# hwwang55/GraphGAN

Measured on NVIDIA B200. Metric: sampled negative edges/sec (D-sampling pass), higher is better.
Workload: dtype f32

## Files before the change

graphgan_b200/_cabi.py:

```python
import ctypes as C
import os

from . import _build

_LIB = None
ABI_VERSION = 3


class GGError(RuntimeError):
    pass


class WalkDesc(C.Structure):
    _fields_ = [
        ("n_node", C.c_int64), ("ld", C.c_int32),
        ("emb", C.c_void_p), ("bias", C.c_void_p), ("indptr", C.c_void_p), ("adj", C.c_void_p),
        ("n_roots", C.c_int64), ("roots", C.c_void_p), ("tree_bits", C.c_void_p), ("tree_words", C.c_int64),
        ("walk_ptr", C.c_void_p),
        ("n_walks", C.c_int64), ("for_d", C.c_int32), ("rng_mode", C.c_int32), ("d1_bits", C.c_void_p),
        ("seed", C.c_uint64), ("pass_tag", C.c_uint32), ("max_path", C.c_int32),
        ("stream", C.c_void_p), ("n_stream", C.c_int64), ("update_ratio", C.c_double),
        ("max_cand", C.c_int32), ("phase_mask", C.c_int32),
        ("samples", C.c_void_p), ("status", C.c_void_p), ("first_edge", C.c_void_p), ("wsteps", C.c_void_p),
        ("wsuml", C.c_void_p), ("paths", C.c_void_p), ("path_len", C.c_void_p), ("counters", C.c_void_p),
        ("scratch", C.c_void_p), ("scratch_bytes", C.c_int64), ("work_counter", C.c_void_p),
        ("edge_score", C.c_void_p), ("root_q", C.c_void_p), ("rq_ptr", C.c_void_p),
        ("hub_threshold", C.c_int32), ("no_tma", C.c_int32), ("walk_slot", C.c_void_p),
        ("s1_nq", C.c_int64), ("s1_slot", C.c_void_p), ("s1_ptr", C.c_void_p), ("s1_cnt", C.c_void_p), ("s1_n", C.c_void_p),
        ("s1_q", C.c_void_p), ("s1_ids", C.c_void_p), ("first_idx", C.c_void_p), ("s1_order", C.c_void_p), ("walk_order", C.c_void_p),
        ("flat_buf", C.c_void_p), ("flat_bytes", C.c_int64), ("flat_steps", C.c_int32), ("flat_reserved", C.c_int32),
    ]


_P, _I32, _I64, _F = C.c_void_p, C.c_int32, C.c_int64, C.c_float
SIGNATURES = {
    "gg_last_error": (C.c_char_p, []),
    "gg_abi_version": (C.c_int, []),
    "gg_hub_scores": (C.c_int, [_I64, _P, _P, _I32, _P, _P, _P, _P, _I32, _P, _P]),
    "gg_root_cdf": (C.c_int, [C.POINTER(WalkDesc), _P, _P, _P]),
    "gg_walk_scratch_bytes": (C.c_int, [_I32, C.POINTER(_I64)]),
    "gg_walk_flat_bytes": (C.c_int, [_I64, _I32, _I32, C.POINTER(_I64)]),
    "gg_walk_sample": (C.c_int, [C.POINTER(WalkDesc), _P]),
    "gg_walk_finalize": (C.c_int, [_I64, _P, _I32, _P, _P, _P, _P, _P, _P, _P, _P, _P, _P]),
    "gg_emit_d_rows": (C.c_int, [_I64, _P, _P, _P, _P, _P, _P, _P, _P, _P, _P, _P, _P]),
    "gg_bfs_scratch_bytes": (C.c_int, [_I64, _I64, C.POINTER(_I64)]),
    "gg_tree_words": (C.c_int, [_I64, C.POINTER(_I64)]),
    "gg_bfs_build": (C.c_int, [_I64, _I64, _P, _P, _I64, _P, _P, _I64, _P, _I64, _P]),
    "gg_reverse_entries": (C.c_int, [_I64, _I64, _P, _P, _P, _P, _P]),
    "gg_bfs_build_ex": (C.c_int, [_I64, _I64, _P, _P, _P, _I64, _P, _P, _I64, _P, _I64, C.c_float, C.c_int32, _P]),
    "gg_tree_parent": (C.c_int, [_I64, _P, _P, _I64, _P, _P, _I64, _P, _P]),
    "gg_pair_reward": (C.c_int, [_I64, _P, _P, _P, _P, _I32, _P, _P]),
    "gg_all_score": (C.c_int, [_I64, _P, _P, _I32, _P, _P]),
    "gg_pair_grad": (C.c_int, [_I32, _I32, _I32, _P, _P, _P, _P, _P, _I32, _F, _P, _P, _P, _P, _P, _P]),
    "gg_grad_buf_floats": (_I64, [_I32, _I32]),
    "gg_grad_merge": (C.c_int, [_I32, _I32, _I32, _P, _P, _P, _P, _P, _P, _P]),
    "gg_comm_unique_id": (C.c_int, [_P]),
    "gg_comm_init": (C.c_int, [_P, _I32, _I32, C.POINTER(C.c_void_p)]),
    "gg_comm_destroy": (C.c_int, [_P]),
    "gg_comm_info": (C.c_int, [_P, C.POINTER(_I32), C.POINTER(_I32), C.POINTER(_I32), C.POINTER(C.c_uint64)]),
# ... 58 lines not shown
```

graphgan_b200/csrc/walk.cu:

```cuda
#include <string.h>

#include "walk_common.cuh"

namespace gg {
namespace {

struct Rng {
    int mode;
    uint32_t k0, k1, tag;
    const double *stream;
    long long n_stream;
    long long cursor;
    int exhausted;
    __device__ __forceinline__ double draw(uint32_t root, uint32_t walk, uint32_t step) {
        if (mode == GG_RNG_PHILOX) {
            uint32_t a, b;
            philox4x32_10(root, walk, step, tag, k0, k1, a, b);
            return u53(a, b);
        }
        if (cursor >= n_stream) { exhausted = 1; return 0.0; }
        return stream[cursor++];
    }
};

// ... 208 lines not shown
            const double u = rng.draw((uint32_t)root, k, (uint32_t)step);
            if (rng.exhausted) { status = GG_NOTRUN; break; }
            idx = (n == 1) ? 0 : choose_index(sc, n, m, u, lane, sc != s_sc ? reinterpret_cast<double *>(s_sc) : nullptr);
            nxt = ids[idx];
            __syncwarp();
            cyc[2] += (unsigned int)(clock64() - t_c);
        }
        cyc[step == 0 ? 3 : (step == 1 ? 4 : 5)] += (unsigned int)(clock64() - t_step);
        if (step == 0) fedge = (int)(a0 + idx);
        if (prow && lane == 0 && plen < d.max_path) prow[plen] = nxt;
        ++plen;
        ++steps; suml += n;
        if (inc_father && idx == 0) { sample = cur; status = GG_DONE; break; }
        prev = cur; cur = nxt; ++step;
    }
    cyc[6] += (unsigned int)(clock64() - t_walk);
    raw_steps += (unsigned)(steps - steps_in); raw_suml += (unsigned)(suml - suml_in);
    if (lane == 0) {
        d.samples[w] = sample;
        d.status[w] = status;
        d.first_edge[w] = fedge;
        d.wsteps[w] = steps;
        d.wsuml[w] = suml;
        if (d.path_len) d.path_len[w] = (status == GG_DONE) ? plen : 0;
    }
    if (status == GG_DONE && d.max_path > 0 && plen > d.max_path) overflow += 1;
    return status;
}

__global__ void root_step_kernel(const __grid_constant__ gg_walk_desc d) {
    const long long w = (long long)blockIdx.x * blockDim.x + threadIdx.x;
    if (w >= d.n_walks) return;
    const int slot = __ldg(d.walk_slot + w);
    const int root = d.roots[slot];
    const uint32_t k = (uint32_t)(w - __ldg(d.walk_ptr + slot));
    const uint32_t k0 = (uint32_t)d.seed, k1 = (uint32_t)(d.seed >> 32);
    uint32_t a, b;
    if (d.update_ratio < 1.0) {
        philox4x32_10((uint32_t)root, 0xffffffffu, 0u, d.pass_tag, k0, k1, a, b);
        if (!(u53(a, b) < d.update_ratio)) { d.first_idx[w] = -2; return; }
    }
    const long long a0 = d.indptr[root];
    const int n = (int)(d.indptr[root + 1] - a0);
    if (n == 0) { d.first_idx[w] = -1; return; }
    philox4x32_10((uint32_t)root, k, 0u, d.pass_tag, k0, k1, a, b);
    const long long o = __ldg(d.rq_ptr + slot);
    const int idx = cdf_search(d.root_q + o, n, u53(a, b));
    d.first_idx[w] = idx;
    atomicAdd(d.s1_cnt + o + idx, 1);
}

constexpr int S1_SINGLES = 8192, S1_CHUNK = 16;

template <int CPL>
__global__ void __launch_bounds__(WARPS_PER_CTA * 32, WALK_MIN_CTAS) step1_cdf_kernel(const __grid_constant__ gg_walk_desc d) {
    extern __shared__ __align__(16) unsigned char walk_smem[];
    const int lane = threadIdx.x & 31, wid = threadIdx.x >> 5;
    float *s_sc = reinterpret_cast<float *>(walk_smem + (size_t)wid * WALK_SMEM_PER_WARP);
    int *s_ids = reinterpret_cast<int *>(s_sc + SC_CAP);
    Stage stg;
    stg.buf = s_sc;
    stg.bar = reinterpret_cast<unsigned long long *>(s_ids + ID_CAP);
    stg.phase = 0u;
    stg.on = !d.no_tma && d.edge_score != nullptr;
    if (stg.on) {
        if (lane == 0) {
            mbar_init(stg.bar, 1);
            asm volatile("fence.mbarrier_init.release.cluster;" ::: "memory");
        }
        __syncwarp();
    }
    const long long gw = (long long)blockIdx.x * WARPS_PER_CTA + wid;
    const long long nwarps = (long long)gridDim.x * WARPS_PER_CTA;
    int *g_ids = reinterpret_cast<int *>(d.scratch) + (size_t)gw * 2 * (size_t)d.max_cand;
    float *g_sc = reinterpret_cast<float *>(g_ids + d.max_cand);
    unsigned long long rows_gathered = 0;
    unsigned int cyc[7] = {0, 0, 0, 0, 0, 0, 0};
    long long item = gw, sub = 0, sub_end = 0;
    const long long n_single = d.s1_nq < S1_SINGLES ? d.s1_nq : S1_SINGLES;
    const long long n_items = n_single + (d.s1_nq - n_single + S1_CHUNK - 1) / S1_CHUNK;
    for (;;) {
        long long pos;
        if (d.s1_order) {
            if (sub >= sub_end) {
                unsigned int it = 0;
                if (lane == 0) it = atomicAdd(d.work_counter, 1u);
                it = __shfl_sync(FULL, it, 0);
                if ((long long)it >= n_items) break;
                if ((long long)it < n_single) { sub = it; sub_end = sub + 1; }
                else { sub = n_single + ((long long)it - n_single) * S1_CHUNK; sub_end = sub + S1_CHUNK < d.s1_nq ? sub + S1_CHUNK : d.s1_nq; }
            }
            pos = __ldg(d.s1_order + sub);
            ++sub;
        } else {
            if (item >= d.s1_nq) break;
            pos = item;
            item += nwarps;
        }
        if (!s1_is_shared(d, pos)) continue;
        const int slot = __ldg(d.s1_slot + pos);
        const int root = d.roots[slot];
        const uint32_t *tb = d.tree_bits + (size_t)slot * (size_t)d.tree_words;
        const long long e = d.indptr[root] + (pos - __ldg(d.rq_ptr + slot));
        const int c = __ldg(d.adj + e);
        const bool inc_father = !d.for_d && !((d.d1_bits[e >> 5] >> (e & 31)) & 1u);
        int n; float m; int *ids; float *sc;
        build_list<CPL, UNR_S1>(d, tb, c, root, inc_father, s_ids, s_sc, g_ids, g_sc, lane, n, m, ids, sc, rows_gathered, cyc, stg);
        if (lane == 0) d.s1_n[pos] = n;
        if (n == 0) continue;
        const long long o = __ldg(d.s1_ptr + pos);
        for (int i = lane; i < n; i += 32) d.s1_ids[o + i] = ids[i];
        if (n > 1) cdf_store_raw<UNR_S1>(sc, n, m, d.s1_q + o, lane);
        __syncwarp();
    }
    if (lane == 0 && rows_gathered) atomicAdd(d.counters + GG_CNT_ROWS_GATHERED, rows_gathered);
}

struct FlatView {
    int4 *list[2];
    int4 *tail;
    int *hub;
    int *item_n;
    int *pool_ids;
    unsigned *ctr;
    int stride;
    int steps;
};
constexpr int FLAT_MAX_STEPS = 14;
constexpr int FLAT_CTR_WORDS = 1 + 4 * (FLAT_MAX_STEPS + 2);
#define GG_FCTR(fv, s, k) ((fv).ctr + 1 + 4 * (s) + (k))

template <int CPL>
__global__ void __launch_bounds__(WARPS_PER_CTA * 32, WALK_MIN_CTAS) walk_kernel(const __grid_constant__ gg_walk_desc d,
                                                                                 const FlatView fv, const int tail_mode) {
    extern __shared__ __align__(16) unsigned char walk_smem[];
    const int lane = threadIdx.x & 31, wid = threadIdx.x >> 5;
    float *s_sc = reinterpret_cast<float *>(walk_smem + (size_t)wid * WALK_SMEM_PER_WARP);
    int *s_ids = reinterpret_cast<int *>(s_sc + SC_CAP);
    Stage stg;
    stg.buf = s_sc;
    stg.bar = reinterpret_cast<unsigned long long *>(s_ids + ID_CAP);
    stg.phase = 0u;
    stg.on = !d.no_tma && d.edge_score != nullptr;
    if (stg.on) {
        if (lane == 0) {
            mbar_init(stg.bar, 1);
            asm volatile("fence.mbarrier_init.release.cluster;" ::: "memory");
        }
        __syncwarp();
    }
    const long long gw = (long long)blockIdx.x * WARPS_PER_CTA + wid;
    int *g_ids = reinterpret_cast<int *>(d.scratch) + (size_t)gw * 2 * (size_t)d.max_cand;
    float *g_sc = reinterpret_cast<float *>(g_ids + d.max_cand);
    Rng rng;
    rng.mode = GG_RNG_PHILOX; rng.k0 = (uint32_t)d.seed; rng.k1 = (uint32_t)(d.seed >> 32); rng.tag = d.pass_tag;
    rng.stream = nullptr; rng.n_stream = 0; rng.cursor = 0; rng.exhausted = 0;
    unsigned long long raw_steps = 0, raw_suml = 0, overflow = 0, rows_gathered = 0;
    unsigned int cyc[7] = {0, 0, 0, 0, 0, 0, 0};
    const bool ratio_all = d.update_ratio >= 1.0;

    const long long n_items = tail_mode ? (long long)fv.ctr[0] : d.n_walks;
    for (;;) {
        unsigned int wi = 0;
        if (lane == 0) wi = atomicAdd(d.work_counter, 1u);
        wi = __shfl_sync(FULL, wi, 0);
        if ((long long)wi >= n_items) break;
        if (tail_mode) {
            const int4 rec = fv.tail[wi];
// ... 434 lines not shown
        const long long slot = walk_root_slot(walk_ptr, n_roots, w);
        if (!root_ok[slot]) continue;
        const int r = roots[slot];
        const long long w0 = walk_ptr[slot], k = walk_ptr[slot + 1] - w0, t = w - w0, o = row_ptr[slot];
        center[o + t] = r; neighbor[o + t] = pos_flat[pos_indptr[r] + t]; label[o + t] = 1;
        center[o + k + t] = r; neighbor[o + k + t] = samples[w]; label[o + k + t] = 0;
    }
}

int grid_ctas() { return sm_count() * WALK_MIN_CTAS; }

}
}

extern "C" int gg_walk_scratch_bytes(int32_t max_cand, int64_t *bytes) {
    GG_REQUIRE(bytes && max_cand > 0, "bad arguments");
    const int64_t warps = (int64_t)gg::grid_ctas() * gg::WARPS_PER_CTA;
    *bytes = warps * 2 * (int64_t)max_cand * 4;
    return 0;
}

extern "C" int gg_walk_flat_bytes(int64_t n_walks, int32_t hub_threshold, int32_t flat_steps, int64_t *bytes) {
    GG_REQUIRE(bytes && n_walks >= 0 && hub_threshold > 0 && flat_steps >= 0 && flat_steps <= gg::FLAT_MAX_STEPS, "bad arguments");
    *bytes = (int64_t)gg::flat_layout(nullptr, n_walks, hub_threshold, flat_steps, nullptr);
    return 0;
}

extern "C" int gg_walk_sample(const gg_walk_desc *dp, void *stream) {
    GG_REQUIRE(dp, "null descriptor");
    const gg_walk_desc &d = *dp;
    GG_REQUIRE(d.ld > 0 && d.ld % 32 == 0, "ld must be a positive multiple of 32");
    if (d.n_walks == 0 || d.n_roots == 0) return 0;
    GG_REQUIRE(d.emb && d.bias && d.indptr && d.adj && d.roots && d.tree_bits && d.walk_ptr, "null graph/embedding pointer");
    GG_REQUIRE(d.tree_words > 0, "tree_words missing (gg_tree_words)");
    GG_REQUIRE(d.samples && d.status && d.first_edge && d.wsteps && d.wsuml && d.counters && d.work_counter,
               "null output pointer");
    GG_REQUIRE(d.for_d || d.d1_bits, "G mode needs d1_bits");
    GG_REQUIRE(d.n_walks < (1ll << 32), "too many walks in one call");
    GG_REQUIRE(d.max_cand > 0 && d.scratch, "scratch missing");
    GG_REQUIRE(!d.root_q || d.rq_ptr, "root_q needs rq_ptr");
    GG_REQUIRE(d.max_path >= 0 && (d.max_path == 0 || (d.paths && d.path_len)), "max_path > 0 needs paths and path_len");
    GG_REQUIRE(d.phase_mask >= 0 && d.phase_mask <= 3, "phase_mask must be 0..3");
    GG_REQUIRE(d.update_ratio >= 0.0, "update_ratio must be >= 0");
    GG_REQUIRE(d.rng_mode == GG_RNG_PHILOX || d.rng_mode == GG_RNG_STREAM, "unknown rng_mode");
    {
        const bool any_s1 = d.s1_q || d.s1_ids || d.s1_cnt || d.s1_n || d.s1_ptr || d.s1_slot || d.first_idx || d.s1_order;
        GG_REQUIRE(!any_s1 || (d.s1_q && d.s1_ids && d.s1_cnt && d.s1_n && d.s1_ptr && d.s1_slot && d.first_idx && d.s1_nq > 0),
                   "depth-1 reuse: s1_q, s1_ids, s1_cnt, s1_n, s1_ptr, s1_slot, first_idx and s1_nq go together");
        GG_REQUIRE(!any_s1 || d.rng_mode == GG_RNG_PHILOX, "depth-1 reuse needs GG_RNG_PHILOX");
        GG_REQUIRE(!d.walk_order || d.rng_mode == GG_RNG_PHILOX, "walk_order needs GG_RNG_PHILOX");
    }
    GG_REQUIRE(!d.edge_score || (d.hub_threshold > 0 && d.hub_threshold < gg::SMEM_CAP), "hub_threshold out of range");
    cudaStream_t st = (cudaStream_t)stream;
    GG_CHECK(cudaMemsetAsync(d.work_counter, 0, sizeof(unsigned int), st));
    if (d.n_walks == 0 || d.n_roots == 0) return 0;
    const int cpl = d.ld / 32;
    if (d.rng_mode == GG_RNG_STREAM) {
        GG_REQUIRE(d.stream, "stream mode needs the uniform stream");
        GG_REQUIRE(d.scratch_bytes >= 2ll * d.max_cand * 4, "scratch too small");
        switch (cpl) {
#define GG_STREAM(C)                                                                                                  \
    GG_CHECK(cudaFuncSetAttribute(gg::walk_stream_kernel<C>, cudaFuncAttributeMaxDynamicSharedMemorySize,            \
                                  gg::WALK_SMEM_PER_WARP));                                                          \
    gg::walk_stream_kernel<C><<<1, 32, gg::WALK_SMEM_PER_WARP, st>>>(d)
            case 1: GG_STREAM(1); break;
            case 2: GG_STREAM(2); break;
            case 4: GG_STREAM(4); break;
            case 8: GG_STREAM(8); break;
#undef GG_STREAM
            default: gg::set_error("gg_walk_sample: unsupported ld %d (supported: 32, 64, 128, 256)", d.ld); return 2;
        }
    } else {
        const int ctas = gg::grid_ctas();
        GG_REQUIRE(d.scratch_bytes >= (int64_t)ctas * gg::WARPS_PER_CTA * 2 * d.max_cand * 4, "scratch too small");
        const int pm = d.phase_mask ? d.phase_mask : 3;
        if (d.s1_q && (pm & 1)) {
            GG_REQUIRE(d.root_q && d.walk_slot && d.first_idx && d.s1_cnt && d.s1_n && d.s1_ptr && d.s1_ids && d.s1_slot,
                       "depth-1 reuse needs root_q, walk_slot and the s1_* buffers");
            GG_CHECK(cudaMemsetAsync(d.s1_cnt, 0, sizeof(int32_t) * (size_t)d.s1_nq, st));
            gg::root_step_kernel<<<(unsigned)((d.n_walks + 255) / 256), 256, 0, st>>>(d);
            GG_CHECK(cudaGetLastError());
#define GG_S1(C)                                                                                                      \
    GG_CHECK(cudaFuncSetAttribute(gg::step1_cdf_kernel<C>, cudaFuncAttributeMaxDynamicSharedMemorySize,              \
                                  gg::WARPS_PER_CTA * gg::WALK_SMEM_PER_WARP));                                      \
    gg::step1_cdf_kernel<C><<<ctas, gg::WARPS_PER_CTA * 32, gg::WARPS_PER_CTA * gg::WALK_SMEM_PER_WARP, st>>>(d)
            switch (cpl) {
                case 1: GG_S1(1); break;
                case 2: GG_S1(2); break;
                case 4: GG_S1(4); break;
                case 8: GG_S1(8); break;
                default: gg::set_error("gg_walk_sample: unsupported ld %d (supported: 32, 64, 128, 256)", d.ld); return 2;
            }
#undef GG_S1
            GG_CHECK(cudaGetLastError());
            GG_CHECK(cudaMemsetAsync(d.work_counter, 0, sizeof(unsigned int), st));
        }
        if (!(pm & 2)) return 0;
        gg::FlatView fv;
        memset(&fv, 0, sizeof(fv));
        int tail_mode = 0;
        if (d.flat_steps > 0) {
            GG_REQUIRE(d.s1_q && d.edge_score && d.root_q && d.walk_slot && d.first_idx, "flat_steps needs the depth-1 reuse (s1_*, edge_score, root_q, walk_slot)");
            GG_REQUIRE(d.flat_steps <= gg::FLAT_MAX_STEPS, "flat_steps too large");
            GG_REQUIRE(d.flat_buf && d.flat_bytes >= (int64_t)gg::flat_layout(nullptr, d.n_walks, d.hub_threshold, d.flat_steps, nullptr),
                       "flat_buf too small (gg_walk_flat_bytes)");
            gg::flat_layout(d.flat_buf, d.n_walks, d.hub_threshold, d.flat_steps, &fv);
            GG_CHECK(cudaMemsetAsync(fv.ctr, 0, sizeof(unsigned) * gg::FLAT_CTR_WORDS, st));
// ... 83 lines not shown
```

graphgan_b200/csrc/walk_common.cuh:

```cuda
#pragma once
#include "gg_common.cuh"

namespace gg {

#ifndef GG_SC_CAP
#define GG_SC_CAP 1024
#endif
#ifndef GG_UNR
#define GG_UNR 2
#endif
#ifndef GG_UNR_S1
#define GG_UNR_S1 8
#endif
#ifndef GG_WALK_MIN_CTAS
#define GG_WALK_MIN_CTAS 4
#endif
constexpr int WARPS_PER_CTA = 8;
constexpr int WALK_MIN_CTAS = GG_WALK_MIN_CTAS;
constexpr int ID_CAP = 320;
constexpr int SC_CAP = GG_SC_CAP;
constexpr int SMEM_CAP = ID_CAP;
constexpr int WALK_SMEM_PER_WARP = SC_CAP * 4 + ID_CAP * 4 + 16;
constexpr int STAGE_ENTRIES = 512;
static_assert(2 * STAGE_ENTRIES * 4 <= SC_CAP * 4, "the staging area is the warp's (idle) score buffer");
// ... 40 lines not shown
#pragma unroll
        for (int c = 0; c < CPL; ++c) sb = fma4(c4[c], xb[c], sb);
        sa = group8_sum(sa);
        sb = group8_sum(sb);
        if (g == 0) {
            if (va) sc[ia] = __fadd_rn(sa, ba);
            if (vb) sc[ib] = __fadd_rn(sb, bb);
        }
    }
    __syncwarp();
}

template <int CPL>
__device__ __forceinline__ void score_edges(const float *__restrict__ emb, const float *__restrict__ bias, int ld,
                                            const float4 (&c4)[CPL], const int *__restrict__ adj, long long e0,
                                            int n, float *out, int fallback, int lane) {
    const int grp = lane >> 3, g = lane & 7;
    int ca_n = (grp < n) ? __ldg(adj + e0 + grp) : fallback, cb_n = (4 + grp < n) ? __ldg(adj + e0 + 4 + grp) : fallback;
    for (int i0 = 0; i0 < n; i0 += 8) {
        const int ia = i0 + grp, ib = i0 + 4 + grp;
        const bool va = ia < n, vb = ib < n;
        const int ca = ca_n, cb = cb_n;
        ca_n = (ia + 8 < n) ? __ldg(adj + e0 + ia + 8) : fallback;
        cb_n = (ib + 8 < n) ? __ldg(adj + e0 + ib + 8) : fallback;
        const float *ra = emb + (size_t)ca * (size_t)ld + 4 * g;
        const float *rb = emb + (size_t)cb * (size_t)ld + 4 * g;
        float4 xa[CPL], xb[CPL];
#pragma unroll
        for (int c = 0; c < CPL; ++c) xa[c] = ldg4(ra + 32 * c);
#pragma unroll
        for (int c = 0; c < CPL; ++c) xb[c] = ldg4(rb + 32 * c);
        const float ba = __ldg(bias + ca), bb = __ldg(bias + cb);
        float sa = 0.0f, sb = 0.0f;
#pragma unroll
        for (int c = 0; c < CPL; ++c) sa = fma4(c4[c], xa[c], sa);
#pragma unroll
        for (int c = 0; c < CPL; ++c) sb = fma4(c4[c], xb[c], sb);
        sa = group8_sum(sa);
        sb = group8_sum(sb);
        if (g == 0) {
            if (va) out[ia] = __fadd_rn(sa, ba);
            if (vb) out[ib] = __fadd_rn(sb, bb);
        }
    }
    __syncwarp();
}

__device__ __forceinline__ float list_max(const float *sc, int n, int lane) {
    float m = -INFINITY;
    for (int i = lane; i < n; i += 32) m = fmaxf(m, sc[i]);
    return warp_max(m);
}

template <int U = UNR>
__device__ __forceinline__ float softmax_exp_sum(float *sc, int n, float m, int lane) {
    float S = 0.0f;
    for (int t0 = 0; t0 < n; t0 += 32 * U) {
        float x[U];
#pragma unroll
        for (int u = 0; u < U; ++u) { const int i = t0 + 32 * u + lane; x[u] = (i < n) ? sc[i] : 0.0f; }
#pragma unroll
        for (int u = 0; u < U; ++u) {
            if (t0 + 32 * u >= n) break;
            const int i = t0 + 32 * u + lane;
            float e = 0.0f;
            if (i < n) { e = exp_c(__fsub_rn(x[u], m)); sc[i] = e; }
            S = __fadd_rn(S, warp_sum_butterfly(e));
        }
    }
    __syncwarp();
    return S;
}

template <int U = UNR>
__device__ __forceinline__ double cdf_total(const float *sc, int n, float S, int lane, double (&car)[2]) {
    double total = 0.0;
    car[0] = car[1] = 0.0;
    for (int t0 = 0; t0 < n; t0 += 32 * U) {
        float e[U];
#pragma unroll
        for (int u = 0; u < U; ++u) { const int i = t0 + 32 * u + lane; e[u] = (i < n) ? sc[i] : 0.0f; }
#pragma unroll
        for (int u = 0; u < U; ++u) {
            if (t0 + 32 * u >= n) break;
            double x = (double)__fdiv_rn(e[u], S);
            x = warp_scan_ks(x, lane);
            total = __dadd_rn(total, __shfl_sync(FULL, x, 31));
            const int t = (t0 >> 5) + u;
            if (t < 64 && lane == (t & 31)) car[t >> 5] = total;
        }
    }
    return total;
}

__device__ __forceinline__ int cdf_pick_from(const float *sc, int n, float S, double total, double u, int lane,
                                             int t_begin, double carry) {
    for (int t0 = 32 * t_begin; t0 < n; t0 += 32) {
        const int i = t0 + lane;
        double x = (double)__fdiv_rn((i < n) ? sc[i] : 0.0f, S);
        x = warp_scan_ks(x, lane);
        const double q = __ddiv_rn(__dadd_rn(carry, x), total);
        const unsigned hit = __ballot_sync(FULL, (i < n) && (q > u));
        if (hit) return t0 + __ffs(hit) - 1;
        carry = __dadd_rn(carry, __shfl_sync(FULL, x, 31));
    }
    return n - 1;
}

__device__ __forceinline__ int cdf_pick(const float *sc, int n, float S, double total, double u, int lane,
                                        const double (&car)[2]) {
    const int ntiles = (n + 31) >> 5;
    int t_hit = -1;
#pragma unroll
    for (int h = 0; h < 2; ++h) {
        const int t = 32 * h + lane;
        const bool p = (t < ntiles) && (__ddiv_rn(car[h], total) > u);
        const unsigned mk = __ballot_sync(FULL, p);
        if (t_hit < 0 && mk) t_hit = 32 * h + __ffs(mk) - 1;
    }
    if (t_hit < 0) {
        if (ntiles <= 64) return n - 1;
        const double c63 = __shfl_sync(FULL, car[1], 31);
        return cdf_pick_from(sc, n, S, total, u, lane, 64, c63);
    }
    double before = 0.0;
    if (t_hit > 0) {
        const int tp = t_hit - 1;
        const double lo = __shfl_sync(FULL, car[0], tp & 31), hi = __shfl_sync(FULL, car[1], tp & 31);
        before = (tp >> 5) ? hi : lo;
    }
    return cdf_pick_from(sc, n, S, total, u, lane, t_hit, before);
}

__device__ __forceinline__ double cdf_total_tiles(const float *sc, int n, float S, int lane, double *tiles) {
    constexpr int U = 8;
    double total = 0.0;
    for (int t0 = 0; t0 < n; t0 += 32 * U) {
        float e[U];
#pragma unroll
        for (int u = 0; u < U; ++u) { const int i = t0 + 32 * u + lane; e[u] = (i < n) ? sc[i] : 0.0f; }
#pragma unroll
        for (int u = 0; u < U; ++u) {
            if (t0 + 32 * u >= n) break;
            double x = (double)__fdiv_rn(e[u], S);
            x = warp_scan_ks(x, lane);
            total = __dadd_rn(total, __shfl_sync(FULL, x, 31));
            if (lane == 0) tiles[(t0 >> 5) + u] = total;
        }
    }
    __syncwarp();
    return total;
}
__device__ __forceinline__ int cdf_pick_tiles(const float *sc, int n, float S, double total, double u, int lane,
                                              const double *tiles) {
    const int ntiles = (n + 31) >> 5;
    for (int tb = 0; tb < ntiles; tb += 32) {
        const int t = tb + lane;
        const bool p = (t < ntiles) && (__ddiv_rn(tiles[t], total) > u);
        const unsigned mk = __ballot_sync(FULL, p);
        if (mk) {
            const int t_hit = tb + __ffs(mk) - 1;
            return cdf_pick_from(sc, n, S, total, u, lane, t_hit, t_hit > 0 ? tiles[t_hit - 1] : 0.0);
        }
    }
    return n - 1;
}

static __device__ __noinline__ int choose_index_long(float *sc, int n, float m, double u, int lane, double *tiles) {
    float S;
    double car[2], total;
    if (tiles && ((n + 31) >> 5) <= SC_CAP / 2) {
        S = softmax_exp_sum<8>(sc, n, m, lane);
        total = cdf_total_tiles(sc, n, S, lane, tiles);
        return cdf_pick_tiles(sc, n, S, total, u, lane, tiles);
    }
    S = softmax_exp_sum<8>(sc, n, m, lane);
    total = cdf_total<8>(sc, n, S, lane, car);
    return cdf_pick(sc, n, S, total, u, lane, car);
}

__device__ __forceinline__ int choose_index(float *sc, int n, float m, double u, int lane, double *tiles = nullptr) {
    if (n <= 32) {
        const float e = (lane < n) ? exp_c(__fsub_rn(sc[lane], m)) : 0.0f;
        const float S = warp_sum_butterfly(e);
        const double x = warp_scan_ks((double)__fdiv_rn(e, S), lane);
        const double total = __shfl_sync(FULL, x, 31);
        const unsigned hit = __ballot_sync(FULL, (lane < n) && (__ddiv_rn(x, total) > u));
        return hit ? __ffs(hit) - 1 : n - 1;
    }
    if (n > SC_CAP) return choose_index_long(sc, n, m, u, lane, tiles);
    double car[2];
    const float S = softmax_exp_sum(sc, n, m, lane);
    const double total = cdf_total(sc, n, S, lane, car);
    return cdf_pick(sc, n, S, total, u, lane, car);
}

__device__ __forceinline__ void cdf_store(float *sc, int n, double *q_out, int lane) {
    const float m = list_max(sc, n, lane);
    const float S = softmax_exp_sum<UNR_S1>(sc, n, m, lane);
    double car[2];
// ... 56 lines not shown
```

graphgan_b200/sampler.py:

```python
import ctypes as C
import os

import numpy as np

from . import _cabi
from ._cabi import ptr

RNG_PHILOX, RNG_STREAM = 0, 1
NOTRUN, DONE, VOID, SKIPPED = 0, 1, 2, 3
CNT = dict(steps=0, sum_l=1, accepted=2, ok_roots=3, path_overflow=4, raw_steps=5, raw_sum_l=6, stream_used=7,
           rows_gathered=8, cyc_enum=9, cyc_score=10, cyc_choose=11, cyc_step0=12, cyc_step1=13, cyc_step2p=14, cyc_walk=15)


def round_up(x, m):
    return (x + m - 1) // m * m


def pad_embedding(emb, device=None):
    import torch
    e = emb.float() if isinstance(emb, torch.Tensor) else torch.as_tensor(np.asarray(emb, np.float64).astype(np.float32))
    n, d = e.shape
    if d > 256:
        raise ValueError("n_emb = %d is not supported (the kernels are instantiated for row strides 32, 64, 128, 256)" % d)
    ld = 32
    while ld < d:
        ld *= 2
    out = torch.zeros((n, ld), dtype=torch.float32, device=device if device is not None else e.device)
    out[:, :d] = e.to(out.device)
    return out


class TreeBatch:

    def __init__(self, roots, tree_bits, graph=None):
        self.roots = roots
        self.tree_bits = tree_bits
        self.graph = graph

    def slice(self, lo, hi):
        return TreeBatch(self.roots[lo:hi].contiguous(), self.tree_bits[lo:hi].contiguous(), self.graph)

    def select(self, idx):
        return TreeBatch(self.roots[idx].contiguous(), self.tree_bits[idx].contiguous(), self.graph)

    def parent_arrays(self, rows=None):
        import torch
        g, lib = self.graph, _cabi.lib()
        bits = self.tree_bits if rows is None else self.tree_bits[rows].contiguous()
        roots = self.roots if rows is None else self.roots[rows].contiguous()
        R = int(bits.shape[0])
        out = torch.empty((R, g.n_node), dtype=torch.int32, device=bits.device)
        st = torch.cuda.current_stream(bits.device).cuda_stream
        for lo in range(0, R, 32768):
            hi = min(R, lo + 32768)
            _cabi.check(lib.gg_tree_parent(g.n_node, ptr(g.indptr), ptr(g.adj), hi - lo, ptr(roots[lo:hi]), ptr(bits[lo:hi]),
                                           int(bits.shape[1]), ptr(out[lo:hi]), st), "gg_tree_parent")
        return out


class WalkOutput:

    def __init__(self, **kw):
        self.__dict__.update(kw)

    def counters_host(self):
        c = self.counters.cpu().numpy().astype(np.uint64)
        return {k: int(c[i]) for k, i in CNT.items()}


class WalkPlan:

    def __init__(self, sampler, trees, sample_num, for_d, max_path):
        import torch
        dev, g = sampler.device, sampler.g
        R = int(trees.roots.shape[0])
        self.trees, self.for_d, self.max_path, self.n_roots = trees, bool(for_d), int(max_path), R
        if isinstance(sample_num, int):
            self.walk_ptr = torch.arange(R + 1, dtype=torch.int64, device=dev) * sample_num
            self.n_walks = R * sample_num
        else:
            self.walk_ptr = torch.zeros(R + 1, dtype=torch.int64, device=dev)
            self.walk_ptr[1:] = torch.cumsum(sample_num.to(torch.int64), 0)
            self.n_walks = int(self.walk_ptr[-1].item())
        nw = self.walk_ptr[1:] - self.walk_ptr[:-1]
        self.walk_slot = torch.repeat_interleave(torch.arange(R, dtype=torch.int32, device=dev), nw,
                                                 output_size=self.n_walks) if self.n_walks else None
        r = trees.roots.long()
        self.rq_ptr = torch.zeros(R + 1, dtype=torch.int64, device=dev)
        self.rq_ptr[1:] = torch.cumsum(g.indptr[r + 1] - g.indptr[r], 0)
        self.nq = int(self.rq_ptr[-1].item())
        nq = max(self.nq, 1)
        self.root_q = torch.empty(nq, dtype=torch.float64, device=dev)
        self.root_sc = torch.empty(nq, dtype=torch.float32, device=dev)
        self._s1 = None
        self._order = None
        W = max(self.n_walks, 1)
        i32 = lambda *s: torch.empty(s, dtype=torch.int32, device=dev)
        self.samples, self.status, self.first_edge, self.wsteps, self.wsuml = i32(W), i32(W), i32(W), i32(W), i32(W)
        self.paths = i32(W, max_path) if max_path > 0 else None
        self.path_len = i32(W) if max_path > 0 else None
        self.root_ok = torch.zeros(max(R, 1), dtype=torch.int32, device=dev)
        self.counters = torch.zeros(16, dtype=torch.int64, device=dev)
        self.row_ptr = torch.empty(R + 1, dtype=torch.int64, device=dev)
        self.n_rows = torch.zeros(1, dtype=torch.int64, device=dev)
        self.rows = [i32(max(2 * self.n_walks, 1)) for _ in range(3)] if for_d else None


    def start_order(self, sampler):
        if self._order is None and self.n_walks > 0 and self.nq > 0:
            torch, g, dev = sampler.torch, sampler.g, sampler.device
            R = self.n_roots
            deg_r = self.rq_ptr[1:] - self.rq_ptr[:-1]
            slot = torch.repeat_interleave(torch.arange(R, dtype=torch.int64, device=dev), deg_r, output_size=self.nq)
            ent = g.indptr[self.trees.roots.long()[slot]] + (torch.arange(self.nq, dtype=torch.int64, device=dev) - self.rq_ptr[slot])
            c = g.adj[ent].long()
            key = torch.zeros(R, dtype=torch.int64, device=dev).scatter_reduce_(0, slot, g.indptr[c + 1] - g.indptr[c], "amax")
            perm = torch.argsort(key, descending=True, stable=True)
            nw = (self.walk_ptr[1:] - self.walk_ptr[:-1])[perm]
            first = torch.cumsum(nw, 0) - nw
            base = torch.repeat_interleave(self.walk_ptr[:-1][perm] - first, nw, output_size=self.n_walks)
            self._order = (base + torch.arange(self.n_walks, dtype=torch.int64, device=dev)).to(torch.int32)
        return self._order

    def flat_buffer(self, sampler):
        key = (sampler.flat_steps, sampler.hub_threshold)
        if getattr(self, "_flat_key", None) != key:
            nbytes = C.c_int64(0)
            _cabi.check(sampler.lib.gg_walk_flat_bytes(self.n_walks, sampler.hub_threshold, sampler.flat_steps, C.byref(nbytes)),
                        "gg_walk_flat_bytes")
            self._flat = sampler.torch.empty(max(nbytes.value, 16), dtype=sampler.torch.uint8, device=sampler.device)
            self._flat_key = key
        return self._flat

    def depth1_buffers(self, sampler):
        if self._s1 is None:
            torch, g, dev = sampler.torch, sampler.g, sampler.device
            deg_r = self.rq_ptr[1:] - self.rq_ptr[:-1]
            slot = torch.repeat_interleave(torch.arange(self.n_roots, dtype=torch.int32, device=dev), deg_r, output_size=self.nq)
            r = self.trees.roots.long()[slot.long()]
            ent = g.indptr[r] + (torch.arange(self.nq, dtype=torch.int64, device=dev) - self.rq_ptr[slot.long()])
            c = g.adj[ent].long()
            ptr_ = torch.zeros(self.nq + 1, dtype=torch.int64, device=dev)
            ptr_[1:] = torch.cumsum(g.indptr[c + 1] - g.indptr[c] + 1, 0)
            total = max(int(ptr_[-1].item()), 1)
            i32 = lambda k: torch.empty(max(k, 1), dtype=torch.int32, device=dev)
            order = torch.argsort(g.indptr[c + 1] - g.indptr[c], descending=True, stable=True).to(torch.int32)
            self._s1 = dict(slot=slot, ptr=ptr_, cnt=i32(self.nq), n=i32(self.nq), ids=i32(total), order=order,
                            q=torch.empty(total, dtype=torch.float64, device=dev), first=i32(self.n_walks))
        return self._s1


class WalkSampler:
    def __init__(self, graph, hub_threshold=128, depth1=True, hub_first=True, tma=True):
        import torch
        self.torch = torch
        self.g = graph
        self.device = graph.device
        self.lib = _cabi.lib()
        self.max_cand = graph.max_deg + 1
        self.hub_threshold = int(hub_threshold)
        self.depth1 = bool(depth1)
        self.tma = bool(tma)
        self.hub_first = bool(hub_first)
        nbytes = C.c_int64(0)
        _cabi.check(self.lib.gg_walk_scratch_bytes(self.max_cand, C.byref(nbytes)), "gg_walk_scratch_bytes")
        self.scratch = torch.empty(max(nbytes.value, 16), dtype=torch.uint8, device=self.device)
        self.work_counter = torch.zeros(1, dtype=torch.int32, device=self.device)
        self._bfs_scratch = None
        self.bfs_bottom_up_ratio = float(os.environ.get("GG_BFS_BU_RATIO", "-1"))
        self.bfs_flags = 0
        self.flat_steps = int(os.environ.get("GG_FLAT_STEPS", "4"))

    def _stream(self):
        return self.torch.cuda.current_stream(self.device).cuda_stream

    def build_trees(self, roots):
        torch = self.torch
        roots_d = roots if isinstance(roots, torch.Tensor) else torch.as_tensor(np.asarray(roots, np.int32)).to(self.device)
        R, N = int(roots_d.shape[0]), self.g.n_node
        nnz = int(self.g.adj.shape[0])
        words = C.c_int64(0)
        _cabi.check(self.lib.gg_tree_words(nnz, C.byref(words)), "gg_tree_words")
        tree_bits = torch.empty((R, words.value), dtype=torch.int32, device=self.device)
        if self._bfs_scratch is None:
            nbytes = C.c_int64(0)
            _cabi.check(self.lib.gg_bfs_scratch_bytes(N, int(self.g.adj.shape[0]), C.byref(nbytes)), "gg_bfs_scratch_bytes")
            self._bfs_scratch = torch.empty(max(nbytes.value, 16), dtype=torch.uint8, device=self.device)
        rev = self.g.reverse_entries() if self.bfs_bottom_up_ratio != 0.0 else None
        _cabi.check(self.lib.gg_bfs_build_ex(N, nnz, ptr(self.g.indptr), ptr(self.g.adj), ptr(rev) if rev is not None else None,
                                             R, ptr(roots_d), ptr(tree_bits), words.value, ptr(self._bfs_scratch),
                                             self._bfs_scratch.numel(), float(self.bfs_bottom_up_ratio), int(self.bfs_flags),
                                             self._stream()),
                    "gg_bfs_build_ex")
        return TreeBatch(roots_d, tree_bits, self.g)

    def plan(self, trees, sample_num, for_d, max_path=0):
        return WalkPlan(self, trees, sample_num, for_d, max_path)

    def _desc(self, emb, bias, plan, *, seed, pass_tag, update_ratio, rng_mode, stream, reuse, phase_mask=0):
        torch = self.torch
        assert emb.dtype == torch.float32 and emb.is_contiguous() and bias.dtype == torch.float32
        t, d = plan.trees, _cabi.WalkDesc()
        d.n_node, d.ld = self.g.n_node, int(emb.shape[1])
        d.emb, d.bias, d.indptr, d.adj = ptr(emb), ptr(bias), ptr(self.g.indptr), ptr(self.g.adj)
        d.n_roots, d.roots, d.walk_ptr, d.n_walks = plan.n_roots, ptr(t.roots), ptr(plan.walk_ptr), plan.n_walks
        d.tree_bits, d.tree_words = ptr(t.tree_bits), int(t.tree_bits.shape[1])
        d.for_d, d.rng_mode, d.d1_bits = int(plan.for_d), rng_mode, ptr(self.g.d1_bits)
        d.seed, d.pass_tag, d.max_path = seed, pass_tag, plan.max_path
        d.stream, d.n_stream = (ptr(stream), int(stream.numel())) if stream is not None else (None, 0)
        d.update_ratio, d.max_cand, d.phase_mask = float(update_ratio), self.max_cand, int(phase_mask)
        d.no_tma = 0 if self.tma else 1
        d.samples, d.status, d.first_edge, d.wsteps, d.wsuml = (ptr(plan.samples), ptr(plan.status), ptr(plan.first_edge),
                                                                 ptr(plan.wsteps), ptr(plan.wsuml))
        d.paths, d.path_len, d.counters = ptr(plan.paths), ptr(plan.path_len), ptr(plan.counters)
        d.scratch, d.scratch_bytes, d.work_counter = ptr(self.scratch), self.scratch.numel(), ptr(self.work_counter)
        d.rq_ptr, d.walk_slot = ptr(plan.rq_ptr), ptr(plan.walk_slot)
        if self.hub_first and rng_mode == RNG_PHILOX:
            d.walk_order = ptr(plan.start_order(self))
        if reuse:
            self.g.hub_tiles(self.hub_threshold)
# ... 56 lines not shown
```

include/graphgan_b200.h:

```cpp
#ifndef GRAPHGAN_B200_H
#define GRAPHGAN_B200_H
#include <stdint.h>

#ifdef __cplusplus
extern "C" {
#endif

#define GG_ABI_VERSION 3

enum { GG_NOTRUN = 0, GG_DONE = 1, GG_VOID = 2, GG_SKIPPED = 3 };
enum {
    GG_RNG_PHILOX = 0,
    GG_RNG_STREAM = 1
};
enum {
    GG_CNT_STEPS = 0, GG_CNT_SUML = 1, GG_CNT_ACCEPTED = 2, GG_CNT_OK_ROOTS = 3,
    GG_CNT_PATH_OVERFLOW = 4, GG_CNT_RAW_STEPS = 5, GG_CNT_RAW_SUML = 6, GG_CNT_STREAM_USED = 7,
    GG_CNT_ROWS_GATHERED = 8,
    GG_CNT_CYC_ENUM = 9, GG_CNT_CYC_SCORE = 10, GG_CNT_CYC_CHOOSE = 11, GG_CNT_CYC_STEP0 = 12,
    GG_CNT_CYC_STEP1 = 13, GG_CNT_CYC_STEP2P = 14, GG_CNT_CYC_WALK = 15,
    GG_CNT_SLOTS = 16
};

const char *gg_last_error(void);
int gg_abi_version(void);

typedef struct gg_walk_desc {
    int64_t n_node;
    int32_t ld;
    const float *emb;
    const float *bias;
    const int64_t *indptr;
    const int32_t *adj;
    int64_t n_roots;
    const int32_t *roots;
    const uint32_t *tree_bits;
    int64_t tree_words;
    const int64_t *walk_ptr;
    int64_t n_walks;
    int32_t for_d;
    int32_t rng_mode;
    uint32_t *d1_bits;
    uint64_t seed;
    uint32_t pass_tag;
    int32_t max_path;
    const double *stream;
    int64_t n_stream;
    double update_ratio;
    int32_t max_cand;
    int32_t phase_mask;
    int32_t *samples;
    int32_t *status;
    int32_t *first_edge;
    int32_t *wsteps;
    int32_t *wsuml;
    int32_t *paths;
    int32_t *path_len;
    unsigned long long *counters;
    void *scratch;
    int64_t scratch_bytes;
    unsigned int *work_counter;
    const float *edge_score;
    const double *root_q;
    const int64_t *rq_ptr;
    int32_t hub_threshold;
    int32_t no_tma;
    const int32_t *walk_slot;
    int64_t s1_nq;
    const int32_t *s1_slot;
    const int64_t *s1_ptr;
    int32_t *s1_cnt;
    int32_t *s1_n;
    double *s1_q;
    int32_t *s1_ids;
// ... 117 lines not shown
```

Before: 120.2 million.

## Build step-1 CDFs for very large neighbor lists cooperatively across a whole CTA

Adds a CTA-cooperative phase in step1_cdf_kernel. Before the per-warp loop, whole blocks claim step-1 items whose neighbor list has at least 2048 entries (via a second work counter) and build their softmax CDF together: they count tree bits per warp, enumerate and score in parallel, then reduce and scan tiles in shared memory. The per-warp path then skips those lists. Separately, the per-warp softmax sum and CDF tile totals switch from one shuffle reduction per 32-element tile to a transposed multi-tile reduction, which needs fewer shuffles. The extra phase adds __syncthreads and a serial thread-0 loop over tiles, moves the mbarrier location in shared memory, and changes the float summation order.

Result: faster. 128.8 million, median of 6 (+7.2%).

```diff
diff --git a/graphgan_b200/_cabi.py b/graphgan_b200/_cabi.py
--- a/graphgan_b200/_cabi.py
+++ b/graphgan_b200/_cabi.py
@@ -4,7 +4,7 @@
 from . import _build
 
 _LIB = None
-ABI_VERSION = 3
+ABI_VERSION = 4
 
 
 class GGError(RuntimeError):
diff --git a/graphgan_b200/csrc/walk.cu b/graphgan_b200/csrc/walk.cu
--- a/graphgan_b200/csrc/walk.cu
+++ b/graphgan_b200/csrc/walk.cu
@@ -284,15 +284,191 @@
 
 constexpr int S1_SINGLES = 8192, S1_CHUNK = 16;
 
+#ifndef GG_CTA_LIST_MIN
+#define GG_CTA_LIST_MIN 2048
+#endif
+constexpr int CTA_LIST_MIN = GG_CTA_LIST_MIN;
+constexpr int CTA_SMEM = WARPS_PER_CTA * (SC_CAP + ID_CAP) * 4;
+constexpr int CTA_G = 8;
+static_assert(CTA_LIST_MIN >= ID_CAP, "CTA lists must be score-cached (hub_threshold < ID_CAP)");
+static_assert(CTA_SMEM + WARPS_PER_CTA * 8 <= WARPS_PER_CTA * WALK_SMEM_PER_WARP, "step1_cdf_kernel layout: buffers, then mbarriers");
+
+__device__ __forceinline__ bool cta_list(const gg_walk_desc &d, long long len) {
+    const long long groups = (len + 1 + 32 * CTA_G - 1) / (32 * CTA_G);
+    return d.edge_score && len >= CTA_LIST_MIN && groups * CTA_G * 8 <= CTA_SMEM;
+}
+
+struct CtaCtl {
+    long long a0, a1, o;
+    int pos, slot, cur, prev, inc_father;
+    int wcnt[WARPS_PER_CTA];
+    float wmax[WARPS_PER_CTA];
+    float S;
+};
+
+template <int CPL>
+__device__ __noinline__ void cta_build_cdf(const gg_walk_desc &d, CtaCtl &ctl, unsigned char *smem, float *g_sc, int lane,
+                                              int wid, unsigned long long &rows_gathered) {
+    const long long a0 = ctl.a0, a1 = ctl.a1;
+    const int f = ctl.inc_father;
+    const uint32_t *tb = d.tree_bits + (size_t)ctl.slot * (size_t)d.tree_words;
+    int *ids = d.s1_ids + ctl.o;
+    double *c_out = d.s1_q + ctl.o;
+    const long long wfirst = a0 >> 5, wlast = (a1 - 1) >> 5;
+    const long long per = (wlast - wfirst + WARPS_PER_CTA) / WARPS_PER_CTA;
+    const long long e_lo = max(a0, (wfirst + wid * per) << 5), e_hi = min(a1, (wfirst + (wid + 1) * per) << 5);
+    int cnt = 0;
+    if (e_lo < e_hi) {
+        const long long wl0 = e_lo >> 5, wl1 = (e_hi - 1) >> 5;
+        for (long long wb = wl0; wb <= wl1; wb += 32) {
+            const long long wi = wb + lane;
+            unsigned word = (wi <= wl1) ? __ldg(tb + wi) : 0u;
+            if (wi == wl0) word &= 0xffffffffu << (e_lo & 31);
+            if (wi == wl1 && (e_hi & 31)) word &= (1u << (e_hi & 31)) - 1u;
+            cnt += (int)__reduce_add_sync(FULL, (unsigned)__popc(word));
+        }
+    }
+    if (lane == 0) ctl.wcnt[wid] = cnt;
+    __syncthreads();
+    int off = f, n = f;
+#pragma unroll
+    for (int w = 0; w < WARPS_PER_CTA; ++w) {
+        const int c = ctl.wcnt[w];
+        if (w < wid) off += c;
+        n += c;
+    }
+    const int ntiles = (n + 31) >> 5;
+    double *tt = reinterpret_cast<double *>(smem);
+    float *sc = ((long long)ntiles * 8 + (long long)n * 4 <= CTA_SMEM) ? reinterpret_cast<float *>(smem + (size_t)ntiles * 8) : g_sc;
+    float m = -INFINITY;
+    if (e_lo < e_hi) {
+        Stage plain;
+        plain.buf = nullptr; plain.bar = nullptr; plain.phase = 0u; plain.on = false;
+        int nloc = 0;
+        enumerate_children<UNR_S1>(d, tb, e_lo, e_hi, true, ids + off, sc + off, lane, nloc, m, plain);
+    }
+    m = warp_max(m);
+    if (f && wid == 0) {
+        if (lane == 0) ids[0] = ctl.prev;
+        if (n > 1) {
+            float4 c4[CPL];
+            load_row<CPL>(d.emb, d.ld, ctl.cur, lane & 7, c4);
+            score_list<CPL>(d.emb, d.bias, d.ld, c4, &ctl.prev, sc, 1, ctl.cur, lane);
+            rows_gathered += 2;
+            m = fmaxf(m, sc[0]);
+        }
+    }
+    if (lane == 0) ctl.wmax[wid] = m;
+    __syncthreads();
+    if (n <= 1) {
+        if (threadIdx.x == 0) d.s1_n[ctl.pos] = n;
+        return;
+    }
+#pragma unroll
+    for (int w = 0; w < WARPS_PER_CTA; ++w) m = fmaxf(m, ctl.wmax[w]);
+    const int ngroups = (ntiles + CTA_G - 1) / CTA_G;
+    float *tsum = reinterpret_cast<float *>(smem);
+    for (int g = wid; g < ngroups; g += WARPS_PER_CTA) {
+        const int i0 = g * 32 * CTA_G;
+        float e[CTA_G];
+#pragma unroll
+        for (int u = 0; u < CTA_G; ++u) { const int i = i0 + 32 * u + lane; e[u] = (i < n) ? sc[i] : 0.0f; }
+#pragma unroll
+        for (int u = 0; u < CTA_G; ++u) {
+            const int i = i0 + 32 * u + lane;
+            if (i < n) { e[u] = exp_c(__fsub_rn(e[u], m)); sc[i] = e[u]; }
+        }
+        const float T = tile_sums<CTA_G>(e, lane);
+        const int t = g * CTA_G + lane / (32 / CTA_G);
+        if (lane % (32 / CTA_G) == 0 && t < ntiles) tsum[t] = T;
+    }
+    __syncthreads();
+    if (threadIdx.x == 0) {
+        float S = 0.0f;
+        for (int t = 0; t < ntiles; ++t) S = __fadd_rn(S, tsum[t]);
+        ctl.S = S;
+    }
+    __syncthreads();
+    const float S = ctl.S;
+    for (int g = wid; g < ngroups; g += WARPS_PER_CTA) {
+        const int i0 = g * 32 * CTA_G;
+        double x[CTA_G];
+#pragma unroll
+        for (int u = 0; u < CTA_G; ++u) { const int i = i0 + 32 * u + lane; x[u] = (double)__fdiv_rn((i < n) ? sc[i] : 0.0f, S); }
+        const double U = tile_totals<CTA_G>(x, lane);
+        const int t = g * CTA_G + tile_total_lane<CTA_G>(lane & (CTA_G - 1));
+        if (lane < CTA_G && t < ntiles) tt[t] = U;
+    }
+    __syncthreads();
+    if (threadIdx.x == 0) {
+        double C = 0.0;
+        for (int t = 0; t < ntiles; ++t) { C = __dadd_rn(C, tt[t]); tt[t] = C; }
+        c_out[n] = C;
+    }
+    __syncthreads();
+    for (int g = wid; g < ngroups; g += WARPS_PER_CTA) {
+        const int i0 = g * 32 * CTA_G;
+        double x[CTA_G];
+#pragma unroll
+        for (int u = 0; u < CTA_G; ++u) { const int i = i0 + 32 * u + lane; x[u] = (i < n) ? (double)__fdiv_rn(sc[i], S) : 0.0; }
+#pragma unroll
+        for (int u = 0; u < CTA_G; ++u) x[u] = warp_scan_ks(x[u], lane);
+#pragma unroll
+        for (int u = 0; u < CTA_G; ++u) {
+            const int t = g * CTA_G + u, i = i0 + 32 * u + lane;
+            if (i < n) c_out[i] = __dadd_rn(t > 0 ? tt[t - 1] : 0.0, x[u]);
+        }
+    }
+    if (threadIdx.x == 0) d.s1_n[ctl.pos] = n;
+}
+
+template <int CPL>
+__device__ __noinline__ unsigned long long cta_phase_run(const gg_walk_desc &d, unsigned char *walk_smem, int lane, int wid,
+                                                       unsigned long long &rows_gathered) {
+    __shared__ CtaCtl ctl;
+    unsigned long long cta_lists = 0;
+    float *cta_sc = reinterpret_cast<float *>(reinterpret_cast<int *>(d.scratch) +
+                                              (size_t)blockIdx.x * WARPS_PER_CTA * 2 * (size_t)d.max_cand + d.max_cand);
+    for (;;) {
+        if (threadIdx.x == 0) {
+            int pos = -1;
+            for (;;) {
+                const unsigned it = atomicAdd(d.work_counter + 1, 1u);
+                if ((long long)it >= d.s1_nq) break;
+                const int p = __ldg(d.s1_order + it);
+                const int slot = __ldg(d.s1_slot + p);
+                const int root = d.roots[slot];
+                const long long e = d.indptr[root] + (p - __ldg(d.rq_ptr + slot));
+                const int c = __ldg(d.adj + e);
+                const long long a0 = d.indptr[c], a1 = d.indptr[c + 1];
+                if (a1 - a0 < CTA_LIST_MIN) break;
+                if (!cta_list(d, a1 - a0) || !s1_is_shared(d, p)) continue;
+                ctl.a0 = a0; ctl.a1 = a1; ctl.o = __ldg(d.s1_ptr + p);
+                ctl.slot = slot; ctl.cur = c; ctl.prev = root;
+                ctl.inc_father = !d.for_d && !((d.d1_bits[e >> 5] >> (e & 31)) & 1u);
+                pos = p;
+                break;
+            }
+            ctl.pos = pos;
+        }
+        __syncthreads();
+        if (ctl.pos < 0) break;
+        cta_build_cdf<CPL>(d, ctl, walk_smem, cta_sc, lane, wid, rows_gathered);
+        cta_lists += 1;
+        __syncthreads();
+    }
+    return cta_lists;
+}
+
 template <int CPL>
 __global__ void __launch_bounds__(WARPS_PER_CTA * 32, WALK_MIN_CTAS) step1_cdf_kernel(const __grid_constant__ gg_walk_desc d) {
     extern __shared__ __align__(16) unsigned char walk_smem[];
     const int lane = threadIdx.x & 31, wid = threadIdx.x >> 5;
-    float *s_sc = reinterpret_cast<float *>(walk_smem + (size_t)wid * WALK_SMEM_PER_WARP);
+    float *s_sc = reinterpret_cast<float *>(walk_smem + (size_t)wid * (SC_CAP + ID_CAP) * 4);
     int *s_ids = reinterpret_cast<int *>(s_sc + SC_CAP);
     Stage stg;
     stg.buf = s_sc;
-    stg.bar = reinterpret_cast<unsigned long long *>(s_ids + ID_CAP);
+    stg.bar = reinterpret_cast<unsigned long long *>(walk_smem + CTA_SMEM) + wid;
     stg.phase = 0u;
     stg.on = !d.no_tma && d.edge_score != nullptr;
     if (stg.on) {
@@ -306,8 +482,10 @@
     const long long nwarps = (long long)gridDim.x * WARPS_PER_CTA;
     int *g_ids = reinterpret_cast<int *>(d.scratch) + (size_t)gw * 2 * (size_t)d.max_cand;
     float *g_sc = reinterpret_cast<float *>(g_ids + d.max_cand);
-    unsigned long long rows_gathered = 0;
+    unsigned long long rows_gathered = 0, cta_lists = 0;
     unsigned int cyc[7] = {0, 0, 0, 0, 0, 0, 0};
+    const bool cta_phase = d.s1_order && d.edge_score;
+    if (cta_phase) cta_lists = cta_phase_run<CPL>(d, walk_smem, lane, wid, rows_gathered);
     long long item = gw, sub = 0, sub_end = 0;
     const long long n_single = d.s1_nq < S1_SINGLES ? d.s1_nq : S1_SINGLES;
     const long long n_items = n_single + (d.s1_nq - n_single + S1_CHUNK - 1) / S1_CHUNK;
@@ -335,6 +513,7 @@
         const uint32_t *tb = d.tree_bits + (size_t)slot * (size_t)d.tree_words;
         const long long e = d.indptr[root] + (pos - __ldg(d.rq_ptr + slot));
         const int c = __ldg(d.adj + e);
+        if (cta_phase && cta_list(d, d.indptr[c + 1] - d.indptr[c])) continue;
         const bool inc_father = !d.for_d && !((d.d1_bits[e >> 5] >> (e & 31)) & 1u);
         int n; float m; int *ids; float *sc;
         build_list<CPL, UNR_S1>(d, tb, c, root, inc_father, s_ids, s_sc, g_ids, g_sc, lane, n, m, ids, sc, rows_gathered, cyc, stg);
@@ -346,6 +525,7 @@
         __syncwarp();
     }
     if (lane == 0 && rows_gathered) atomicAdd(d.counters + GG_CNT_ROWS_GATHERED, rows_gathered);
+    if (threadIdx.x == 0 && cta_lists) atomicAdd(d.counters + GG_CNT_CTA_LISTS, cta_lists);
 }
 
 struct FlatView {
@@ -886,7 +1066,7 @@
     }
     GG_REQUIRE(!d.edge_score || (d.hub_threshold > 0 && d.hub_threshold < gg::SMEM_CAP), "hub_threshold out of range");
     cudaStream_t st = (cudaStream_t)stream;
-    GG_CHECK(cudaMemsetAsync(d.work_counter, 0, sizeof(unsigned int), st));
+    GG_CHECK(cudaMemsetAsync(d.work_counter, 0, 2 * sizeof(unsigned int), st));
     if (d.n_walks == 0 || d.n_roots == 0) return 0;
     const int cpl = d.ld / 32;
     if (d.rng_mode == GG_RNG_STREAM) {
diff --git a/graphgan_b200/csrc/walk_common.cuh b/graphgan_b200/csrc/walk_common.cuh
--- a/graphgan_b200/csrc/walk_common.cuh
+++ b/graphgan_b200/csrc/walk_common.cuh
@@ -116,21 +116,68 @@
     return warp_max(m);
 }
 
+template <int G, typename T, typename Add>
+__device__ __forceinline__ T transposed_levels(T (&v)[G], int lane, int o0, bool down, Add add) {
+    static_assert(G >= 1 && G <= 32 && (G & (G - 1)) == 0, "G must be a power of two <= 32");
+    int o = o0;
+#pragma unroll
+    for (int k = G; k > 1; k >>= 1) {
+        const bool up = (lane & o) != 0;
+#pragma unroll
+        for (int j = 0; j < k / 2; ++j) {
+            const T send = up ? v[j] : v[j + k / 2];
+            const T keep = up ? v[j + k / 2] : v[j];
+            v[j] = add(keep, __shfl_xor_sync(FULL, send, o));
+        }
+        o = down ? (o >> 1) : (o << 1);
+    }
+    return v[0];
+}
+
+template <int G>
+__device__ __forceinline__ float tile_sums(float (&v)[G], int lane) {
+    const auto add = [](float a, float b) { return __fadd_rn(a, b); };
+    float s = transposed_levels<G>(v, lane, 16, true, add);
+#pragma unroll
+    for (int o = 16 / G; o >= 1; o >>= 1) s = __fadd_rn(s, __shfl_xor_sync(FULL, s, o));
+    return s;
+}
+template <int G>
+__device__ __forceinline__ constexpr int tile_sum_lane(int u) { return u * (32 / G); }
+
+template <int G>
+__device__ __forceinline__ double tile_totals(double (&v)[G], int lane) {
+    const auto add = [](double a, double b) { return __dadd_rn(a, b); };
+    double s = transposed_levels<G>(v, lane, 1, false, add);
+#pragma unroll
+    for (int o = G; o < 32; o <<= 1) s = __dadd_rn(s, __shfl_xor_sync(FULL, s, o));
+    return s;
+}
+template <int G>
+__device__ __forceinline__ constexpr int tile_total_lane(int u) {
+    int r = 0;
+    for (int b = 1, rb = G >> 1; b < G; b <<= 1, rb >>= 1) if (u & b) r |= rb;
+    return r;
+}
+
 template <int U = UNR>
 __device__ __forceinline__ float softmax_exp_sum(float *sc, int n, float m, int lane) {
     float S = 0.0f;
     for (int t0 = 0; t0 < n; t0 += 32 * U) {
-        float x[U];
-#pragma unroll
-        for (int u = 0; u < U; ++u) { const int i = t0 + 32 * u + lane; x[u] = (i < n) ? sc[i] : 0.0f; }
-#pragma unroll
-        for (int u = 0; u < U; ++u) {
-            if (t0 + 32 * u >= n) break;
+        float e[U];
+#pragma unroll
+        for (int u = 0; u < U; ++u) { const int i = t0 + 32 * u + lane; e[u] = (i < n) ? sc[i] : 0.0f; }
+#pragma unroll
+        for (int u = 0; u < U; ++u) {
             const int i = t0 + 32 * u + lane;
-            float e = 0.0f;
-            if (i < n) { e = exp_c(__fsub_rn(x[u], m)); sc[i] = e; }
-            S = __fadd_rn(S, warp_sum_butterfly(e));
-        }
+            if (i < n) { e[u] = exp_c(__fsub_rn(e[u], m)); sc[i] = e[u]; }
+        }
+        const float T = tile_sums<U>(e, lane);
+        float Tu[U];
+#pragma unroll
+        for (int u = 0; u < U; ++u) Tu[u] = __shfl_sync(FULL, T, tile_sum_lane<U>(u));
+#pragma unroll
+        for (int u = 0; u < U; ++u) S = __fadd_rn(S, Tu[u]);
     }
     __syncwarp();
     return S;
@@ -141,15 +188,16 @@
     double total = 0.0;
     car[0] = car[1] = 0.0;
     for (int t0 = 0; t0 < n; t0 += 32 * U) {
-        float e[U];
-#pragma unroll
-        for (int u = 0; u < U; ++u) { const int i = t0 + 32 * u + lane; e[u] = (i < n) ? sc[i] : 0.0f; }
-#pragma unroll
-        for (int u = 0; u < U; ++u) {
-            if (t0 + 32 * u >= n) break;
-            double x = (double)__fdiv_rn(e[u], S);
-            x = warp_scan_ks(x, lane);
-            total = __dadd_rn(total, __shfl_sync(FULL, x, 31));
+        double x[U];
+#pragma unroll
+        for (int u = 0; u < U; ++u) { const int i = t0 + 32 * u + lane; x[u] = (double)__fdiv_rn((i < n) ? sc[i] : 0.0f, S); }
+        const double Ut = tile_totals<U>(x, lane);
+        double Uu[U];
+#pragma unroll
+        for (int u = 0; u < U; ++u) Uu[u] = __shfl_sync(FULL, Ut, tile_total_lane<U>(u));
+#pragma unroll
+        for (int u = 0; u < U; ++u) {
+            total = __dadd_rn(total, Uu[u]);
             const int t = (t0 >> 5) + u;
             if (t < 64 && lane == (t & 31)) car[t >> 5] = total;
         }
@@ -200,16 +248,17 @@
     constexpr int U = 8;
     double total = 0.0;
     for (int t0 = 0; t0 < n; t0 += 32 * U) {
-        float e[U];
-#pragma unroll
-        for (int u = 0; u < U; ++u) { const int i = t0 + 32 * u + lane; e[u] = (i < n) ? sc[i] : 0.0f; }
-#pragma unroll
-        for (int u = 0; u < U; ++u) {
-            if (t0 + 32 * u >= n) break;
-            double x = (double)__fdiv_rn(e[u], S);
-            x = warp_scan_ks(x, lane);
-            total = __dadd_rn(total, __shfl_sync(FULL, x, 31));
-            if (lane == 0) tiles[(t0 >> 5) + u] = total;
+        double x[U];
+#pragma unroll
+        for (int u = 0; u < U; ++u) { const int i = t0 + 32 * u + lane; x[u] = (double)__fdiv_rn((i < n) ? sc[i] : 0.0f, S); }
+        const double Ut = tile_totals<U>(x, lane);
+        double Uu[U];
+#pragma unroll
+        for (int u = 0; u < U; ++u) Uu[u] = __shfl_sync(FULL, Ut, tile_total_lane<U>(u));
+#pragma unroll
+        for (int u = 0; u < U; ++u) {
+            total = __dadd_rn(total, Uu[u]);
+            if (lane == 0 && t0 + 32 * u < n) tiles[(t0 >> 5) + u] = total;
         }
     }
     __syncwarp();
diff --git a/graphgan_b200/sampler.py b/graphgan_b200/sampler.py
--- a/graphgan_b200/sampler.py
+++ b/graphgan_b200/sampler.py
@@ -9,7 +9,8 @@
 RNG_PHILOX, RNG_STREAM = 0, 1
 NOTRUN, DONE, VOID, SKIPPED = 0, 1, 2, 3
 CNT = dict(steps=0, sum_l=1, accepted=2, ok_roots=3, path_overflow=4, raw_steps=5, raw_sum_l=6, stream_used=7,
-           rows_gathered=8, cyc_enum=9, cyc_score=10, cyc_choose=11, cyc_step0=12, cyc_step1=13, cyc_step2p=14, cyc_walk=15)
+           rows_gathered=8, cyc_enum=9, cyc_score=10, cyc_choose=11, cyc_step0=12, cyc_step1=13, cyc_step2p=14, cyc_walk=15,
+           cta_lists=16)
 
 
 def round_up(x, m):
@@ -100,7 +101,7 @@
         self.paths = i32(W, max_path) if max_path > 0 else None
         self.path_len = i32(W) if max_path > 0 else None
         self.root_ok = torch.zeros(max(R, 1), dtype=torch.int32, device=dev)
-        self.counters = torch.zeros(16, dtype=torch.int64, device=dev)
+        self.counters = torch.zeros(len(CNT), dtype=torch.int64, device=dev)
         self.row_ptr = torch.empty(R + 1, dtype=torch.int64, device=dev)
         self.n_rows = torch.zeros(1, dtype=torch.int64, device=dev)
         self.rows = [i32(max(2 * self.n_walks, 1)) for _ in range(3)] if for_d else None
@@ -165,7 +166,7 @@
         nbytes = C.c_int64(0)
         _cabi.check(self.lib.gg_walk_scratch_bytes(self.max_cand, C.byref(nbytes)), "gg_walk_scratch_bytes")
         self.scratch = torch.empty(max(nbytes.value, 16), dtype=torch.uint8, device=self.device)
-        self.work_counter = torch.zeros(1, dtype=torch.int32, device=self.device)
+        self.work_counter = torch.zeros(2, dtype=torch.int32, device=self.device)
         self._bfs_scratch = None
         self.bfs_bottom_up_ratio = float(os.environ.get("GG_BFS_BU_RATIO", "-1"))
         self.bfs_flags = 0
diff --git a/include/graphgan_b200.h b/include/graphgan_b200.h
--- a/include/graphgan_b200.h
+++ b/include/graphgan_b200.h
@@ -6,7 +6,7 @@
 extern "C" {
 #endif
 
-#define GG_ABI_VERSION 3
+#define GG_ABI_VERSION 4
 
 enum { GG_NOTRUN = 0, GG_DONE = 1, GG_VOID = 2, GG_SKIPPED = 3 };
 enum {
@@ -19,7 +19,8 @@
     GG_CNT_ROWS_GATHERED = 8,
     GG_CNT_CYC_ENUM = 9, GG_CNT_CYC_SCORE = 10, GG_CNT_CYC_CHOOSE = 11, GG_CNT_CYC_STEP0 = 12,
     GG_CNT_CYC_STEP1 = 13, GG_CNT_CYC_STEP2P = 14, GG_CNT_CYC_WALK = 15,
-    GG_CNT_SLOTS = 16
+    GG_CNT_CTA_LISTS = 16,
+    GG_CNT_SLOTS = 17
 };
 
 const char *gg_last_error(void);
```
